# mit-acl/rl_collision_avoidance

Measured on AMD Instinct MI355X. Metric: agent-steps/sec (env.step) at 4 agents x 8192 worlds per GPU, higher is better.
Workload: dtype f64

## Files before the change

### include/cavoid.h

```cpp
#ifndef CAVOID_H
#define CAVOID_H
#include <stdint.h>

#ifdef __cplusplus
extern "C" {
#endif

#define CAVOID_ABI_VERSION 3
#define CAVOID_MAX_ACTIONS 32
#define CAVOID_MAX_AGENTS 64

#define CAVOID_F_AT_GOAL 0x01u
#define CAVOID_F_RAN_OUT 0x02u
#define CAVOID_F_IN_COLL 0x04u
#define CAVOID_F_WAS_AT_GOAL 0x08u
#define CAVOID_F_WAS_IN_COLL 0x10u
#define CAVOID_F_PRESENT 0x20u
#define CAVOID_F_LEARNING 0x40u
#define CAVOID_F_POLICY_SHIFT 8
#define CAVOID_F_POLICY_MASK 7u
enum { CAVOID_POLICY_EXTERNAL = 0, CAVOID_POLICY_STATIC = 1, CAVOID_POLICY_NONCOOP = 2, CAVOID_POLICY_RVO = 3, CAVOID_POLICY_FROZEN_NET = 4 };
#define CAVOID_F_DONE_MASK 0x07u

enum { CAVOID_SORT_CLOSEST_LAST = 0, CAVOID_SORT_CLOSEST_FIRST = 1, CAVOID_SORT_TIME_TO_IMPACT = 2 };
// ... 91 lines not shown
int cavoid_step_autoreset_n(cavoid_env *env, const int32_t *actions, int64_t action_stride, int32_t n_steps, int64_t out_step_stride,
                            float *obs, float *rewards, uint8_t *done, uint8_t *game_over, void *stream);

enum {
    CAVOID_FORM_NONE = 0,
    CAVOID_FORM_STEP = 1,
    CAVOID_FORM_QUAD = 2,
    CAVOID_FORM_RVO = 3,
    CAVOID_FORM_LOOP_PF = 4,
    CAVOID_FORM_LOOP = 5,
    CAVOID_FORM_PIPE = 6,
    CAVOID_FORM_RELAY = 7,
    CAVOID_FORM_CROWD = 8
};
int32_t cavoid_last_step_form(const cavoid_env *env, int32_t *relay_consumers);

int cavoid_step_continuous_autoreset(cavoid_env *env, const float *actions , float *obs, float *rewards, uint8_t *done,
                                     uint8_t *game_over, void *stream);
int cavoid_step_continuous_autoreset_n(cavoid_env *env, const float *actions, int64_t action_stride, int32_t n_steps, int64_t out_step_stride,
                                       float *obs, float *rewards, uint8_t *done, uint8_t *game_over, void *stream);

int32_t cavoid_packed_width(const cavoid_env *env);
int cavoid_reset_packed(cavoid_env *env, const uint8_t *world_mask, float *packed, void *stream);
int cavoid_observe_packed(cavoid_env *env, float *packed, void *stream);
int cavoid_step_packed(cavoid_env *env, const int32_t *actions, float *packed, uint8_t *game_over, void *stream);
int cavoid_step_autoreset_packed(cavoid_env *env, const int32_t *actions, int64_t action_stride, int32_t n_steps, int64_t out_step_stride,
                                 float *packed, uint8_t *game_over, void *stream);
int cavoid_step_continuous_autoreset_packed(cavoid_env *env, const float *actions, int64_t action_stride, int32_t n_steps,
                                            int64_t out_step_stride, float *packed, uint8_t *game_over, void *stream);

// ... 124 lines not shown
```

### rl_collision_avoidance_amd/_lib.py

```python
from __future__ import annotations

import ctypes as C
import os

from .build import LIB_PATH as _DEFAULT_LIB_PATH

LIB_PATH = os.environ.get("CAVOID_LIB", _DEFAULT_LIB_PATH)

MAX_ACTIONS = 32
MAX_AGENTS = 64
TILE_MAX_AGENTS = 16
ABI_VERSION = 3

F_AT_GOAL, F_RAN_OUT, F_IN_COLL, F_WAS_AT_GOAL, F_WAS_IN_COLL, F_PRESENT, F_LEARNING = 1, 2, 4, 8, 16, 32, 64
F_POLICY_SHIFT = 8
F_POLICY_MASK = 7
POLICY_EXTERNAL, POLICY_STATIC, POLICY_NONCOOP, POLICY_RVO, POLICY_FROZEN_NET = 0, 1, 2, 3, 4
F_DONE_MASK = 7
COMM_FORCE_RCCL = 1
STEP_FORMS = ("NONE", "STEP", "QUAD", "RVO", "LOOP_PF", "LOOP", "PIPE", "RELAY", "CROWD")


class CavoidCfg(C.Structure):
    _fields_ = [
# ... 53 lines not shown
        self.code = code


_P = C.c_void_p
SYMBOLS = [
    ("cavoid_abi_version", C.c_int, []),
    ("cavoid_strerror", C.c_char_p, [C.c_int]),
    ("cavoid_last_hip_error", C.c_int, []),
    ("cavoid_default_cfg", C.c_int, [C.POINTER(CavoidCfg), C.c_int32, C.c_int32]),
    ("cavoid_default_actions", C.c_int, [_P, C.POINTER(C.c_int32)]),
    ("cavoid_create", C.c_int, [C.POINTER(CavoidCfg), C.c_int64, C.c_int64, C.c_int, C.POINTER(_P)]),
    ("cavoid_destroy", None, [_P]),
    ("cavoid_num_worlds", C.c_int64, [_P]),
    ("cavoid_obs_width", C.c_int32, [_P]),
    ("cavoid_last_step_form", C.c_int32, [_P, C.POINTER(C.c_int32)]),
    ("cavoid_seed", C.c_int, [_P, C.c_uint64, _P, _P]),
    ("cavoid_get_episode", C.c_int, [_P, _P, _P]),
    ("cavoid_pool_refresh", C.c_int, [_P, C.c_uint32, _P]),
    ("cavoid_set_state", C.c_int, [_P, _P, _P, _P, _P]),
    ("cavoid_get_state", C.c_int, [_P, _P, _P, _P, _P]),
    ("cavoid_reset", C.c_int, [_P, _P, _P, _P]),
    ("cavoid_observe", C.c_int, [_P, _P, _P]),
    ("cavoid_step", C.c_int, [_P, _P, _P, _P, _P, _P, _P]),
    ("cavoid_step_continuous", C.c_int, [_P, _P, _P, _P, _P, _P, _P]),
    ("cavoid_step_autoreset", C.c_int, [_P, _P, _P, _P, _P, _P, _P]),
    ("cavoid_step_autoreset_n", C.c_int, [_P, _P, C.c_int64, C.c_int32, C.c_int64, _P, _P, _P, _P, _P]),
    ("cavoid_step_continuous_autoreset", C.c_int, [_P, _P, _P, _P, _P, _P, _P]),
    ("cavoid_step_continuous_autoreset_n", C.c_int, [_P, _P, C.c_int64, C.c_int32, C.c_int64, _P, _P, _P, _P, _P]),
    ("cavoid_step_continuous_autoreset_packed", C.c_int, [_P, _P, C.c_int64, C.c_int32, C.c_int64, _P, _P, _P]),
    ("cavoid_step_autoreset_n_timed", C.c_int, [_P, _P, C.c_int64, C.c_int32, C.c_int32, C.c_int64, _P, _P, _P, _P, _P, C.POINTER(C.c_float)]),
# ... 73 lines not shown
```

### rl_collision_avoidance_amd/batched_env.py

```python
from __future__ import annotations

import ctypes as C
from typing import Optional, Tuple

import numpy as np
import torch

from . import _lib
from .config import EnvConfig

_SORT = {"closest_last": 0, "closest_first": 1, "time_to_impact": 2}
_DYN = {"unicycle": 0, "unicycle_max_turn_rate": 1, "holonomic": 2}


def make_cfg(config: Optional[EnvConfig] = None, **overrides) -> _lib.CavoidCfg:
    config = config or EnvConfig()
    cfg = _lib.CavoidCfg()
    N = int(config.MAX_NUM_AGENTS_IN_ENVIRONMENT)
    M = int(config.MAX_NUM_OTHER_AGENTS_OBSERVED)
    _lib.check(_lib.lib().cavoid_default_cfg(C.byref(cfg), N, M), "cavoid_default_cfg")
    cfg.dt = config.DT
    cfg.near_goal_threshold = config.NEAR_GOAL_THRESHOLD
    cfg.max_time_ratio = config.MAX_TIME_RATIO
    cfg.collision_dist = config.COLLISION_DIST
# ... 181 lines not shown
    def refresh_pool(self, epoch: int) -> None:
        _lib.check(self._lib.cavoid_pool_refresh(self._h, int(epoch) & 0xFFFFFFFF, self._stream()), "cavoid_pool_refresh")

    @property
    def episode(self) -> torch.Tensor:
        out = torch.empty((self.num_worlds,), dtype=torch.int32, device=self.device)
        _lib.check(self._lib.cavoid_get_episode(self._h, self._ptr(out), self._stream()), "cavoid_get_episode")
        return out

    @property
    def last_step_form(self) -> Tuple[str, int]:
        nc = C.c_int32(0)
        form = self._lib.cavoid_last_step_form(self._h, C.byref(nc))
        return _lib.STEP_FORMS[form], int(nc.value)

    def set_state(self, state_f64: torch.Tensor, state_f32: torch.Tensor, flags: torch.Tensor) -> None:
        A = self.num_worlds * self.max_agents
        f64 = self._want(state_f64, (4, A), torch.float64, "state_f64")
        f32 = self._want(state_f32, (5, A), torch.float32, "state_f32")
        fl = self._want(flags, (A,), torch.int32, "flags")
        _lib.check(self._lib.cavoid_set_state(self._h, self._ptr(f64), self._ptr(f32), self._ptr(fl), self._stream()),
                   "cavoid_set_state")

    def get_state(self) -> Tuple[torch.Tensor, torch.Tensor, torch.Tensor]:
        A = self.num_worlds * self.max_agents
        f64 = torch.empty((4, A), dtype=torch.float64, device=self.device)
        f32 = torch.empty((5, A), dtype=torch.float32, device=self.device)
        fl = torch.empty((A,), dtype=torch.int32, device=self.device)
        _lib.check(self._lib.cavoid_get_state(self._h, self._ptr(f64), self._ptr(f32), self._ptr(fl), self._stream()),
                   "cavoid_get_state")
# ... 164 lines not shown
```

### rl_collision_avoidance_amd/csrc/cavoid_capi.hip

```cpp
#include <hip/hip_runtime.h>
#include <hip/hip_ext.h>

#include <cmath>
#include <cstdlib>
#include <cstring>
#include <new>

#include "cavoid.h"
#include "cavoid_host.hpp"
#include "cavoid_kernels.hpp"
#include "cavoid_launch.hpp"
#include "cavoid_crowd.hpp"

using namespace cavoid;

thread_local int g_last_hip_error = 0;

extern "C" int cavoid_abi_version(void) { return CAVOID_ABI_VERSION; }

extern "C" int cavoid_last_hip_error(void) { return g_last_hip_error; }

extern "C" const char *cavoid_strerror(int code) {
    switch (code) {
        case CAVOID_OK: return "ok";
// ... 312 lines not shown
        return cavoid_launch_rvo(e, MODE, io, s, ev_start, ev_stop);
    if (MODE == MODE_STEP_AUTORESET) {
        const int rc = cavoid_launch_quad(e, io, s, ev_start, ev_stop);
        if (rc != CAVOID_EUNSUPPORTED) return rc;
    }
    const int rc = launch_on<MODE>(e, e->k, e->st, e->grid, io, s, ev_start, ev_stop);
    return stepping ? note_form(e, rc, CAVOID_FORM_STEP) : rc;
}

extern "C" int32_t cavoid_last_step_form(const cavoid_env *e, int32_t *relay_consumers) {
    const int32_t form = e ? e->last_form : CAVOID_FORM_NONE;
    if (relay_consumers) *relay_consumers = form == CAVOID_FORM_RELAY ? e->last_relay_consumers : 0;
    return form;
}

int cavoid_ahead_prepare(cavoid_env *e, int32_t n_steps, hipStream_t s, hipEvent_t *timed_start) {
    if (!e || e->ahead_R <= 0) return CAVOID_OK;
    if (n_steps + 1 > e->ahead_R) return CAVOID_EUNSUPPORTED;
    hipStreamCaptureStatus cap = hipStreamCaptureStatusNone;
    (void)hipStreamIsCapturing(s, &cap);
    const bool capturing = cap != hipStreamCaptureStatusNone;
    if (capturing) e->ahead_always = true;
    if (!e->ahead_always && e->ahead_primed && e->ahead_budget >= n_steps + 1) return CAVOID_OK;
    const int64_t waves = (e->W + e->k.wpw - 1) / e->k.wpw;
    const bool in_place = e->ahead_always;
    const dim3 grid((unsigned)((waves + 3) / 4), in_place ? 1u : (e->ahead_primed ? 4u : 32u)), block(256);
    const uint32_t *hi_in = e->ahead_hi[e->ahead_cur];
    uint32_t *hi_out = e->ahead_hi[in_place ? e->ahead_cur : (e->ahead_cur ^ 1)];
    hipEvent_t ev_fill = (timed_start && !capturing) ? *timed_start : nullptr;
    if (ev_fill) *timed_start = nullptr;
    const int rc = dispatch_n(e->cfg.max_agents, EnvNs{}, [&](auto n) -> int {
        launch_kernel(ahead_fill_kernel<decltype(n)::value>, grid, block, 0, s, ev_fill, nullptr, e->k, e->st.episode, hi_in, hi_out, e->pool, e->ahead_R);
        return CAVOID_OK;
    });
    if (rc != CAVOID_OK) return rc;
    HIP_TRY(hipGetLastError());
    if (!in_place) e->ahead_cur ^= 1;
    if (!capturing) { e->ahead_primed = true; e->ahead_budget = e->ahead_R; }
    return CAVOID_OK;
}
void cavoid_ahead_consumed(cavoid_env *e, int32_t n_steps) {
    if (!e || e->ahead_R <= 0) return;
    e->ahead_budget = e->ahead_budget > n_steps ? e->ahead_budget - n_steps : 0;
}

static int fill_pool(cavoid_env *e, hipStream_t s) {
    if (e->ahead_R > 0) {
        e->ahead_budget = 0;
        e->ahead_primed = false;
        HIP_TRY(hipMemsetAsync(e->ahead_hi[0], 0xFF, 2 * (size_t)e->W * sizeof(uint32_t), s));
        return CAVOID_OK;
    }
    if (e->pool_size <= 0) return CAVOID_OK;
    HIP_TRY(hipMemsetAsync(e->pool_episode, 0xFF, (size_t)e->pool_size * sizeof(uint32_t), s));
    KCfg k = e->k;
    k.num_worlds = e->pool_size;
    k.world_offset = 0;
    k.pool_size = 0;
    KState st{};
// ... 118 lines not shown
    return launch<MODE_STEP>(e, io, static_cast<hipStream_t>(stream));
}

static int launch_autoreset(cavoid_env *e, KIO io, const int32_t *actions, int64_t action_stride, int32_t n_steps, int64_t out_step_stride,
                            hipStream_t s, hipEvent_t ev_start = nullptr, hipEvent_t ev_stop = nullptr, const float *cont = nullptr) {
    if (e->cfg.dynamics == CAVOID_DYN_HOLONOMIC && !cont) return CAVOID_EINVAL;
    if (n_steps < 1 || action_stride < 0) return CAVOID_EINVAL;
    if (cont && n_steps > 1 && action_stride != 0 && action_stride < 2 * e->A) return CAVOID_EINVAL;
    if (out_step_stride != 0 && out_step_stride < e->W) return CAVOID_EINVAL;
    io.out_step_stride = n_steps > 1 ? out_step_stride : 0;
    io.actions = actions;
    io.cont = cont;
    io.action_stride = action_stride;
    io.n_steps = n_steps;
    e->last_form = CAVOID_FORM_NONE;
    if (int rc = cavoid_ahead_prepare(e, n_steps, s, &ev_start)) return rc;
    const int rc = (n_steps > 1 || e->prefetch_single)
                       ? cavoid_launch_multistep(e, io, e->latency_mode != 0, s, ev_start, ev_stop)
                       : launch<MODE_STEP_AUTORESET>(e, io, s, ev_start, ev_stop);
    cavoid_ahead_consumed(e, n_steps);
    return rc;
}

extern "C" int cavoid_step_autoreset(cavoid_env *e, const int32_t *actions, float *obs, float *rew, uint8_t *done, uint8_t *game_over, void *stream) {
    if (step_args(e, actions, rew, done, game_over) != CAVOID_OK) return CAVOID_EINVAL;
    return launch_autoreset(e, plain_io(e, obs, rew, done, game_over), actions, 0, 1, 0, static_cast<hipStream_t>(stream));
}

extern "C" int cavoid_step_autoreset_n(cavoid_env *e, const int32_t *actions, int64_t action_stride, int32_t n_steps, int64_t out_step_stride,
                                       float *obs, float *rew, uint8_t *done, uint8_t *game_over, void *stream) {
    if (step_args(e, actions, rew, done, game_over) != CAVOID_OK || n_steps < 0) return CAVOID_EINVAL;
    if (n_steps == 0) return CAVOID_OK;
    return launch_autoreset(e, plain_io(e, obs, rew, done, game_over), actions, action_stride, n_steps, out_step_stride,
                            static_cast<hipStream_t>(stream));
// ... 119 lines not shown
```

### rl_collision_avoidance_amd/csrc/cavoid_launch.hpp

```cpp
#pragma once
#include <hip/hip_runtime.h>
#include <hip/hip_ext.h>

#include <type_traits>

#include "cavoid.h"
#include "cavoid_host.hpp"
#include "cavoid_kernels.hpp"

struct cavoid_env {
    int device = 0;
    int64_t W = 0, A = 0, world_offset = 0;
    cavoid_cfg cfg{};
    cavoid::KCfg k{};
    cavoid::KState st{};
    cavoid::PoolRec *pool = nullptr;
    uint32_t *pool_episode = nullptr;
    int64_t pool_size = 0;
    int ahead_R = 0;
    uint32_t *ahead_hi[2] = {nullptr, nullptr};
    int ahead_cur = 0;
    int ahead_budget = 0;
    bool ahead_primed = false;
    bool ahead_always = false;
    void *slab = nullptr;
    void *pool_slab = nullptr;
    double *d_actions = nullptr;
    int waves_per_block = 4;
    int grid = 0;
    int pipeline = 2;
    int relay_consumers = 3;
    int latency_mode = 0;
    int quad = -1;
    int prefetch_single = 0;
    int last_form = CAVOID_FORM_NONE;
    int last_relay_consumers = 0;
    hipEvent_t ev0 = nullptr, ev1 = nullptr;
};
// ... 81 lines not shown
    const dim3 grid((unsigned)tiles), block(128);
    const int rc = dispatch_n(e->cfg.max_agents, EnvNs{}, [&](auto n) -> int {
        constexpr int N = decltype(n)::value;
        const size_t lds = pipe_lds_fixed_bytes<N>() + tail;
        if (lds > 65536) return CAVOID_EUNSUPPORTED;
        launch_kernel(env_pipe_kernel<N, RVO>, grid, block, lds, s, ev_start, ev_stop, k, e->st, e->pool, io);
        return CAVOID_OK;
    });
    if (rc != CAVOID_OK) return rc;
    HIP_TRY(hipGetLastError());
    return CAVOID_OK;
}

}

int cavoid_ahead_prepare(cavoid_env *e, int32_t n_steps, hipStream_t s, hipEvent_t *timed_start = nullptr);
void cavoid_ahead_consumed(cavoid_env *e, int32_t n_steps);
int cavoid_launch_relay(cavoid_env *e, const cavoid::KIO &io, hipStream_t s, hipEvent_t ev_start, hipEvent_t ev_stop);
int cavoid_launch_quad(cavoid_env *e, const cavoid::KIO &io, hipStream_t s, hipEvent_t ev_start, hipEvent_t ev_stop);
int cavoid_launch_multistep(cavoid_env *e, const cavoid::KIO &io, bool prefetch, hipStream_t s, hipEvent_t ev_start, hipEvent_t ev_stop);
int cavoid_launch_rvo(cavoid_env *e, int mode, const cavoid::KIO &io, hipStream_t s, hipEvent_t ev_start, hipEvent_t ev_stop);
int cavoid_launch_crowd(cavoid_env *e, int mode, const cavoid::KCfg &k, const cavoid::KState &st, int64_t worlds, const cavoid::KIO &io,
                        hipStream_t s, hipEvent_t ev_start, hipEvent_t ev_stop);
#ifdef CAVOID_TRACE
int cavoid_debug_trace_multistep(unsigned long long *dev_ptr);
int cavoid_debug_trace_rvo(unsigned long long *dev_ptr);
int cavoid_debug_trace_relay(unsigned long long *dev_ptr);
int cavoid_debug_trace_quad(unsigned long long *dev_ptr);
#endif
```

### rl_collision_avoidance_amd/csrc/cavoid_multistep.hip

```cpp
#include "cavoid_launch.hpp"

using namespace cavoid;

int cavoid_launch_multistep(cavoid_env *e, const KIO &io, bool prefetch, hipStream_t s, hipEvent_t ev_start, hipEvent_t ev_stop) {
    if (crowd_form(e->cfg.max_agents))
        return note_form(e, cavoid_launch_crowd(e, MODE_STEP_AUTORESET_N, e->k, e->st, e->W, io, s, ev_start, ev_stop), CAVOID_FORM_CROWD);
    if (e->k.rvo_enabled || (e->k.gen_mode == 1 && e->k.pool_size <= 0))
        return cavoid_launch_rvo(e, prefetch ? MODE_STEP_AUTORESET_PF : MODE_STEP_AUTORESET_N, io, s, ev_start, ev_stop);
    if (prefetch && e->pipeline >= 2 && !io.cont) {
        const int rc = cavoid_launch_relay(e, io, s, ev_start, ev_stop);
        if (rc != CAVOID_EUNSUPPORTED) return rc;
    }
    if (prefetch && e->pipeline && !io.cont) {
        const int rc = launch_pipe<false>(e, io, s, ev_start, ev_stop);
        if (rc != CAVOID_EUNSUPPORTED) return note_form(e, rc, CAVOID_FORM_PIPE);
    }
    if (prefetch) return note_form(e, launch_on<MODE_STEP_AUTORESET_PF>(e, e->k, e->st, e->grid, io, s, ev_start, ev_stop), CAVOID_FORM_LOOP_PF);
    return note_form(e, launch_on<MODE_STEP_AUTORESET_N>(e, e->k, e->st, e->grid, io, s, ev_start, ev_stop), CAVOID_FORM_LOOP);
}

#ifdef CAVOID_TRACE
int cavoid_debug_trace_multistep(unsigned long long *dev_ptr) { return set_trace(dev_ptr); }
#endif
```

### rl_collision_avoidance_amd/csrc/cavoid_relay.hip

```cpp
#include "cavoid_launch.hpp"
#include "cavoid_relay.hpp"

using namespace cavoid;

template <int N>
static int relay_allow_lds() {
    static bool allowed = false;
    if (!allowed) {
        HIP_TRY(hipFuncSetAttribute(reinterpret_cast<const void *>(env_relay_kernel<N>), hipFuncAttributeMaxDynamicSharedMemorySize, (int)kRelayLdsLimit));
        allowed = true;
    }
    return CAVOID_OK;
}

int cavoid_launch_relay(cavoid_env *e, const KIO &io, hipStream_t s, hipEvent_t ev_start, hipEvent_t ev_stop) {
    const KCfg &k = e->k;
    if (k.rvo_enabled || k.pool_size <= 0 || !io.obs || !io.actions || io.cont) return CAVOID_EUNSUPPORTED;
    if (k.switches & kSwSkipDonePairs) return CAVOID_EUNSUPPORTED;
    const int64_t tiles = (e->W + k.wpw - 1) / k.wpw;
    if (tiles > 512) return CAVOID_EUNSUPPORTED;
    if (e->cfg.max_agents > kRelayMaxAgents) return CAVOID_EUNSUPPORTED;
    const int row = io.obs_stride;
    const int tile_floats = (k.tile_rows * row + 3) & ~3;
    if (k.tile_rows < k.wpw * e->cfg.max_agents) return CAVOID_EUNSUPPORTED;
    const dim3 grid((unsigned)tiles);
    int used_nc = 0;
    const int rc = dispatch_n(e->cfg.max_agents, RelayNs{}, [&](auto n) -> int {
        constexpr int N = decltype(n)::value;
        int nc = e->relay_consumers;
        while (nc > 1 && relay_lds_fixed_bytes<N>() + (size_t)nc * tile_floats * sizeof(float) > kRelayLdsLimit) --nc;
        const size_t lds = relay_lds_fixed_bytes<N>() + (size_t)nc * tile_floats * sizeof(float);
        if (lds > kRelayLdsLimit || (nc < 2 && e->relay_consumers >= 2)) return CAVOID_EUNSUPPORTED;
        if (lds > 65536) {
            const int rc_opt = relay_allow_lds<N>();
            if (rc_opt != CAVOID_OK) return rc_opt;
        }
        used_nc = nc;
        launch_kernel(env_relay_kernel<N>, grid, dim3(64 * (3 + nc)), lds, s, ev_start, ev_stop, k, e->st, e->pool, io);
        return CAVOID_OK;
    });
    if (rc != CAVOID_OK) return rc;
    HIP_TRY(hipGetLastError());
    return note_form(e, CAVOID_OK, CAVOID_FORM_RELAY, used_nc);
}

#ifdef CAVOID_TRACE
int cavoid_debug_trace_relay(unsigned long long *dev_ptr) { return set_trace(dev_ptr); }
#endif
```

### rl_collision_avoidance_amd/csrc/cavoid_relay.hpp

```cpp
#pragma once
#include "cavoid_kernels.hpp"

namespace cavoid {

constexpr int kRelayMaxAgents = 6;
template <int N>
__host__ __device__ constexpr int relay_ring() { return N <= 5 ? 8 : 4; }
constexpr size_t kRelayLdsLimit = 80 * 1024;
constexpr int kRelayActRing = 64;
constexpr int kRelayActAhead = 48;
constexpr int kRelayEvq = 8;

struct RelaySeq {
    int spec;
    int stage;
    int res;
    int fin;
    int act;
    int ev;
    int nxt;
    int cons[kRelayMaxConsumers];
    int cfin[kRelayMaxConsumers];
    int coop[2];
    int kernarg[2];
// ... 3 lines not shown
struct RelayTent { double px[64], py[64], vx[64], vy[64], heading[64]; float r[64], gx[64], gy[64], pref[64]; uint32_t flags[64]; };
struct RelayRes { uint32_t flags[64], ctl[64]; float rew[64]; };
struct RelayNxt { double px[64], py[64], heading[64], t_rem[64]; float gx[64], gy[64], radius[64], pref[64]; uint32_t flags[64]; };
#ifndef CAVOID_RELAY_ORDER
#define CAVOID_RELAY_ORDER 0x432150
#endif
#ifndef CAVOID_RELAY_PRIO_D
#define CAVOID_RELAY_PRIO_D 3
#endif
#ifndef CAVOID_RELAY_PRIO_P
#define CAVOID_RELAY_PRIO_P 3
#endif
#ifndef CAVOID_RELAY_PRIO_L
#define CAVOID_RELAY_PRIO_L 0
#endif
#ifndef CAVOID_RELAY_PRIO_C
#define CAVOID_RELAY_PRIO_C 1
#endif
#ifndef CAVOID_RELAY_ABL
#define CAVOID_RELAY_ABL 0
#endif
__device__ __forceinline__ int relay_role_of(int wv, int NC) {
    if (NC == 3) return (int)(((unsigned)CAVOID_RELAY_ORDER >> (4 * wv)) & 15u);
    return wv;
}
constexpr int kRelayCoopWaves = 3;
constexpr int kRelayCoopFromN = 4;
template <int N>
struct RelayCoop {
    static constexpr int K = Others<N>::K;
    uint64_t key[K][64];
    uint32_t bits[K][64];
};
template <int N>
__host__ __device__ constexpr size_t relay_coop_bytes() { return N >= kRelayCoopFromN ? sizeof(RelayCoop<N>) : 0; }
template <int N>
__host__ __device__ constexpr size_t relay_lds_fixed_bytes() {
    return (size_t)lds_floats_block() * sizeof(float) + sizeof(RelaySeq) + kRelayActRing * 64 + relay_ring<N>() * (sizeof(RelayTent) + sizeof(RelayRes)) +
           sizeof(RelayNxt) + kRelayEvq * sizeof(unsigned long long) + relay_coop_bytes<N>();
}

#ifdef CAVOID_TRACE
#define RELAY_STAMP(k)                                                                                         \
    do {                                                                                                       \
        if (lane0 == 0 && g_trace && t == (n_steps >> 1)) g_trace[wave * 32 + (k)] = (unsigned long long)clock64(); \
    } while (0)
#define RELAY_MARK(k)                                                                                          \
    do {                                                                                                       \
        if (lane0 == 0 && g_trace) g_trace[wave * 32 + (k)] = (unsigned long long)clock64();                   \
    } while (0)
#else
#define RELAY_STAMP(k) do { } while (0)
#define RELAY_MARK(k) do { } while (0)
#endif
// ... 184 lines not shown
        gapf[o] = (float)gap_o;
        neighbour_features(e, (float)e.prll_x, (float)e.prll_y, rx, ry, q, feat[o]);
    }
}

struct RelayArgs { KCfg c; KState s; const PoolRec *pool; KIO io; };
template <class T>
__device__ __forceinline__ void relay_load_args(T &dst, const __attribute__((address_space(4))) T *src) {
    static_assert(sizeof(T) % 4 == 0, "whole words");
    const __attribute__((address_space(4))) uint32_t *w = (const __attribute__((address_space(4))) uint32_t *)src;
    uint32_t d[sizeof(T) / 4];
#pragma unroll
    for (int k = 0; k < (int)(sizeof(T) / 4); ++k) d[k] = w[k];
    __builtin_memcpy(&dst, d, sizeof(T));
}
template <int N>
__device__ __forceinline__ void relay_coop_last(unsigned char *smem) {
    unsigned char *sp = smem + lds_floats_block() * sizeof(float);
    RelaySeq *seq = reinterpret_cast<RelaySeq *>(sp); sp += sizeof(RelaySeq) + kRelayEvq * sizeof(unsigned long long);
    const unsigned long long kp = (unsigned long long)(uint32_t)relay_peek(&seq->kernarg[0]) | ((unsigned long long)(uint32_t)relay_peek(&seq->kernarg[1]) << 32);
    typedef const __attribute__((address_space(4))) RelayArgs *ArgP;
    const ArgP ka = (ArgP)kp;
    KCfg c;
    KIO io;
    relay_load_args(c, &ka->c);
    relay_load_args(io, &ka->io);
    RelayTent *tents = reinterpret_cast<RelayTent *>(sp); sp += relay_ring<N>() * sizeof(RelayTent) + sizeof(RelayNxt);
    RelayRes *ress = reinterpret_cast<RelayRes *>(sp); sp += relay_ring<N>() * sizeof(RelayRes) + kRelayActRing * 64;
    RelayCoop<N> *coopb = reinterpret_cast<RelayCoop<N> *>(sp); sp += relay_coop_bytes<N>();
    float *tiles = reinterpret_cast<float *>(sp);
    const int lane0 = threadIdx.x & 63;
    const int NC = (blockDim.x >> 6) - 3;
    const int role = relay_role_of(threadIdx.x >> 6, NC);
    const int pw = role < 2 ? role : 2;
    const int ostride = io.obs_stride;
    const int tile_floats = (c.tile_rows * ostride + 3) & ~3;
    const int wpw = c.wpw, lanes_used = wpw * N;
    const int64_t wave = relay_peek(&seq->tile_id);
    const int64_t w0 = wave * wpw;
    const int lw = lane0 / N, i0 = lane0 - lw * N;
    const int64_t w = w0 + lw;
    const bool active = lane0 < lanes_used && w < c.num_worlds;
// ... 61 lines not shown
        const bool lines = ((rows_active * ostride) & 31) == 0 && (reinterpret_cast<uintptr_t>(dst) & 127) == 0;
        if (io.out_step_stride != 0 && lines) flush_tile<4, true, true>(tile, dst, rows_active * ostride, pw * 64 + lane0, 64 * kRelayCoopWaves);
        else if (io.out_step_stride != 0) flush_tile<4, true>(tile, dst, rows_active * ostride, pw * 64 + lane0, 64 * kRelayCoopWaves);
        else flush_tile<4>(tile, dst, rows_active * ostride, pw * 64 + lane0, 64 * kRelayCoopWaves);
    }
    if (pw == 0 && active) {
        if (!packed) {
            io.rew[slot_w * N + a_idx0] = rew_c;
            io.done[slot_w * N + a_idx0] = (ctl_c & 1u) ? 1 : 0;
        }
        if (i0 == 0) io.game_over[slot_w + w] = (ctl_c & 2u) ? 1 : 0;
    }
    if (pw == 0) RELAY_MARK(29);
}

template <int N>
__global__ void __launch_bounds__(64 * (3 + kRelayMaxConsumers), 1) env_relay_kernel(const KCfg c, const KState s, const PoolRec *pool, const KIO io) {
    extern __shared__ __attribute__((aligned(16))) unsigned char smem[];
    unsigned char *sp = smem;
    double *lds_tab = reinterpret_cast<double *>(sp); sp += lds_floats_block() * sizeof(float);
    RelaySeq *seq = reinterpret_cast<RelaySeq *>(sp); sp += sizeof(RelaySeq);
    unsigned long long *evq = reinterpret_cast<unsigned long long *>(sp); sp += kRelayEvq * sizeof(unsigned long long);
    RelayTent *tents = reinterpret_cast<RelayTent *>(sp); sp += relay_ring<N>() * sizeof(RelayTent);
    RelayNxt *nbuf = reinterpret_cast<RelayNxt *>(sp); sp += sizeof(RelayNxt);
    RelayRes *ress = reinterpret_cast<RelayRes *>(sp); sp += relay_ring<N>() * sizeof(RelayRes);
    unsigned char *actring = sp; sp += kRelayActRing * 64;
    RelayCoop<N> *coopb = reinterpret_cast<RelayCoop<N> *>(sp); sp += relay_coop_bytes<N>();
    float *tiles = reinterpret_cast<float *>(sp);

    const int NC = (blockDim.x >> 6) - 3;
    const int role = relay_role_of(threadIdx.x >> 6, NC);
    const int lane0 = threadIdx.x & 63;
    const int ostride = io.obs_stride;
    const int tile_floats = (c.tile_rows * ostride + 3) & ~3;
    const int wpw = c.wpw, lanes_used = wpw * N;
    const int64_t wave = blockIdx.x;
    const int64_t w0 = wave * wpw;
    const int lw = lane0 / N, i0 = lane0 - lw * N;
    const int64_t w = w0 + lw;
    const bool active = lane0 < lanes_used && w < c.num_worlds;
    const int base0 = lane0 < lanes_used ? lw * N : 0;
    const int64_t a_idx0 = w * N + i0;
    const bool packed = io.packed != 0;
    int64_t worlds_here = c.num_worlds - w0;
    if (worlds_here > wpw) worlds_here = wpw;
    if (worlds_here < 0) worlds_here = 0;
    const int n_steps = io.n_steps;
    constexpr bool kCoop = N >= kRelayCoopFromN;
    const bool coop_role = role < 2 || role == 2 + NC;

    if (role == 0 && lane0 < (int)(sizeof(RelaySeq) / sizeof(int))) reinterpret_cast<int *>(seq)[lane0] = 0;
    if constexpr (kCoop) {
        if (role == 0 && lane0 == 0) {
            const unsigned long long kp = (unsigned long long)__builtin_amdgcn_kernarg_segment_ptr();
            seq->kernarg[0] = (int)(uint32_t)kp; seq->kernarg[1] = (int)(uint32_t)(kp >> 32);
            seq->tile_id = (int)blockIdx.x;
        }
    }

    if (role == 0) {
        __builtin_amdgcn_s_setprio(CAVOID_RELAY_PRIO_D);
        RELAY_MARK(20);
        KCfg cd = c;
        asm volatile("" : "+s"(cd.dt), "+s"(cd.near_goal_sq), "+s"(cd.actions_fp32), "+s"(cd.dynamics),
                     "+s"(cd.timeout_enabled), "+s"(cd.switches));
        const RelayTrig trig = relay_trig_constants();
        Agent a;
// ... 70 lines not shown
            if (CAVOID_RARE((posted >> 1) < t + 1 - ((CAVOID_RELAY_ABL & 16) ? 1 : 0)))
                do posted = relay_peek(&seq->res); while ((posted >> 1) < t + 1 - ((CAVOID_RELAY_ABL & 16) ? 1 : 0));
            asm volatile("" ::: "memory");
            RELAY_STAMP(2);
            moved_any = moved_any || T_moving;
            const bool surprise = !(CAVOID_RELAY_ABL & 24) && (posted >> 1) == t + 1 && (posted & 1) != 0;
            if (CAVOID_RARE(surprise)) {
                const uint32_t vflags = *(relay_lds_u32 *)&res->flags[lane], ctl = *(relay_lds_u32 *)&res->ctl[lane];
                const bool restart = (ctl & 2u) != 0u;
                const unsigned long long rmask = __ballot(restart);
                Agent S = T;
                S.flags = vflags;
                if (rmask != 0ull) {
                    relay_wait(&seq->nxt, events + 1);
                    Agent nx;
                    relay_read_nxt(*nbuf, lane, nx);
                    bool mr;
                    const RelayStatics ksn = relay_statics(nx, active);
                    const Agent Tr = relay_advance(cd, trig, nx, ksn, tab_s1, tab_h1, active, mr);
                    if (restart) {
                        S = nx; episode += 1u; restarted_any = true; Tn = Tr; mn = mr; ks = ksn;
                        stage_out(tents[t & (relay_ring<N>() - 1)], nx, ksn.r_staged, lane);
                        res->flags[lane] = nx.flags;
                    }
                }
                const bool s_present = active && (S.flags & CAVOID_F_PRESENT);
                const bool s_done = (S.flags & CAVOID_F_DONE_MASK) != 0u;
                const bool frozen = s_present && s_done && !restart;
                uint32_t fflags = S.flags;
                if (S.flags & CAVOID_F_AT_GOAL) fflags |= CAVOID_F_WAS_AT_GOAL;
                if (S.flags & CAVOID_F_IN_COLL) fflags |= CAVOID_F_WAS_IN_COLL;
                Tn.px = frozen ? S.px : Tn.px; Tn.py = frozen ? S.py : Tn.py; Tn.heading = frozen ? S.heading : Tn.heading;
                Tn.t_rem = frozen ? S.t_rem : Tn.t_rem;
                Tn.vx = frozen ? 0.0 : Tn.vx; Tn.vy = frozen ? 0.0 : Tn.vy; Tn.speed = frozen ? 0.0f : Tn.speed;
                Tn.flags = frozen ? fflags : Tn.flags;
                mn = frozen ? false : mn;
                stage_out(tn, Tn, ks.r_staged, lane);
                relay_post(&seq->stage, t + 2);
                if (rmask != 0ull) {
                    relay_wait(&seq->nxt, events + 1 - (kRelayEvq - 1));
                    if (lane == 0) evq[events & (kRelayEvq - 1)] = rmask;
                    events += 1;
                    relay_post(&seq->ev, events);
                }
            }
            T = Tn;
            T_moving = mn;
            tab_s = tab_s2; tab_h = tab_h2;
            act_q = act3;
            relay_post(&seq->fin, t + 1);
            RELAY_STAMP(3);
        }
        Agent S = T;
        {
            const int t = n_steps - 1;
            relay_spin(&seq->res, 2 * (t + 1));
            RelayRes *res = &ress[t & (relay_ring<N>() - 1)];
            const uint32_t vflags = res->flags[lane0], ctl = res->ctl[lane0];
            moved_any = moved_any || T_moving;
            S.flags = vflags;
            const bool restart = (ctl & 2u) != 0u;
            if (__ballot(restart) != 0ull) {
                relay_wait(&seq->nxt, events + 1);
                Agent nx;
                relay_read_nxt(*nbuf, lane0, nx);
                if (restart) {
                    S = nx; episode += 1u; restarted_any = true;
                    stage_out(tents[t & (relay_ring<N>() - 1)], nx, relay_statics(nx, active).r_staged, lane0);
                    res->flags[lane0] = nx.flags;
                }
            }
            relay_post(&seq->fin, t + 1);
        }
        RELAY_MARK(23);
        relay_post(&seq->stage, n_steps + 1);
        if (restarted_any) {
            store_agent(s, a_idx0, S);
            if (i0 == 0) s.episode[w] = episode;
        } else if (present_first) {
            if (moved_any) {
// ... 83 lines not shown
                    const int sidx = loaded + q < upto ? loaded + q : upto - 1;
                    v[q] = io.actions[(int64_t)sidx * io.action_stride + a_safe];
                }
#pragma unroll
                for (int q = 0; q < 8; ++q) {
                    int x = v[q] < 0 ? 0 : (v[q] >= c.num_actions ? c.num_actions - 1 : v[q]);
                    if (loaded + q < upto) actring[((loaded + q) & (kRelayActRing - 1)) * 64 + lane0] = (unsigned char)x;
                }
                loaded = loaded + 8 < upto ? loaded + 8 : upto;
            }
        };
        load_actions(n_steps < 8 ? n_steps : 8);
        RELAY_MARK(26);
        __syncthreads();
        relay_post(&seq->act, loaded);
        {
            Agent r0;
            absent_agent(r0);
            if (active) load_pool(pool, (int64_t)pool_index(c, (uint32_t)(c.world_offset + w), ep + 1u) * N + i0, r0);
            RelayNxt &nb = *nbuf;
            nb.px[lane0] = r0.px; nb.py[lane0] = r0.py; nb.heading[lane0] = r0.heading; nb.t_rem[lane0] = r0.t_rem;
            nb.gx[lane0] = r0.gx; nb.gy[lane0] = r0.gy; nb.radius[lane0] = r0.radius; nb.pref[lane0] = r0.pref;
            nb.flags[lane0] = r0.flags;
            relay_post(&seq->nxt, 1);
            RELAY_MARK(27);
        }
        int served = 0, idle_polls = 0;
        while (true) {
            const int ev = relay_peek(&seq->ev), fin = relay_peek(&seq->fin);
            if (served < ev) {
                asm volatile("" ::: "memory");
                const unsigned long long mask = evq[served & (kRelayEvq - 1)];
                if ((mask >> lane0) & 1ull) {
                    ep += 1u;
                    Agent r0;
                    load_pool(pool, (int64_t)pool_index(c, (uint32_t)(c.world_offset + w), ep + 1u) * N + i0, r0);
                    RelayNxt &nb = *nbuf;
                    nb.px[lane0] = r0.px; nb.py[lane0] = r0.py; nb.heading[lane0] = r0.heading; nb.t_rem[lane0] = r0.t_rem;
                    nb.gx[lane0] = r0.gx; nb.gy[lane0] = r0.gy; nb.radius[lane0] = r0.radius; nb.pref[lane0] = r0.pref;
                    nb.flags[lane0] = r0.flags;
                }
                served += 1;
                idle_polls = 0;
                relay_post(&seq->nxt, served + 1);
                continue;
            }
            if (loaded < n_steps && loaded < fin + kRelayActAhead) {
                int upto = fin + kRelayActAhead;
                if (upto > loaded + 8) upto = loaded + 8;
                if (upto > n_steps) upto = n_steps;
                load_actions(upto);
                idle_polls = 0;
                relay_post(&seq->act, loaded);
                continue;
            }
            if (fin >= n_steps && relay_peek(&seq->stage) > n_steps) break;
            if (++idle_polls > kRelayPollLimit) __builtin_trap();
            __builtin_amdgcn_s_sleep(2);
        }
// ... 47 lines not shown
                    io.rew[slot_w * N + a_idx0] = rew_c;
                    io.done[slot_w * N + a_idx0] = (ctl_c & 1u) ? 1 : 0;
                }
                if (i0 == 0) io.game_over[slot_w + w] = (ctl_c & 2u) ? 1 : 0;
            }
            relay_post(&seq->cons[cid], t + 1);
            RELAY_STAMP(19);
            if (t == 0) RELAY_MARK(28);
            if (t == n_steps - 1) RELAY_MARK(29);
        }
        __builtin_amdgcn_s_waitcnt(0);
        if (cid == 0) RELAY_MARK(30);
        relay_post(&seq->cfin[cid], 1);
    }
    if constexpr (kCoop) {
        if (coop_role) relay_coop_last<N>(smem);
    }
}

}
```

Before: 23.62 billion.

## Generate next-episode agents inside relay loader wave instead of reading ahead ring

```diff
diff --git a/include/cavoid.h b/include/cavoid.h
--- a/include/cavoid.h
+++ b/include/cavoid.h
@@ -129,6 +129,7 @@
     CAVOID_FORM_CROWD = 8
 };
 int32_t cavoid_last_step_form(const cavoid_env *env, int32_t *relay_consumers);
+int64_t cavoid_ahead_refills(const cavoid_env *env);
 
 int cavoid_step_continuous_autoreset(cavoid_env *env, const float *actions , float *obs, float *rewards, uint8_t *done,
                                      uint8_t *game_over, void *stream);
diff --git a/rl_collision_avoidance_amd/_lib.py b/rl_collision_avoidance_amd/_lib.py
--- a/rl_collision_avoidance_amd/_lib.py
+++ b/rl_collision_avoidance_amd/_lib.py
@@ -91,6 +91,7 @@
     ("cavoid_num_worlds", C.c_int64, [_P]),
     ("cavoid_obs_width", C.c_int32, [_P]),
     ("cavoid_last_step_form", C.c_int32, [_P, C.POINTER(C.c_int32)]),
+    ("cavoid_ahead_refills", C.c_int64, [_P]),
     ("cavoid_seed", C.c_int, [_P, C.c_uint64, _P, _P]),
     ("cavoid_get_episode", C.c_int, [_P, _P, _P]),
     ("cavoid_pool_refresh", C.c_int, [_P, C.c_uint32, _P]),
diff --git a/rl_collision_avoidance_amd/batched_env.py b/rl_collision_avoidance_amd/batched_env.py
--- a/rl_collision_avoidance_amd/batched_env.py
+++ b/rl_collision_avoidance_amd/batched_env.py
@@ -219,6 +219,10 @@
         form = self._lib.cavoid_last_step_form(self._h, C.byref(nc))
         return _lib.STEP_FORMS[form], int(nc.value)
 
+    @property
+    def ahead_refills(self) -> int:
+        return int(self._lib.cavoid_ahead_refills(self._h))
+
     def set_state(self, state_f64: torch.Tensor, state_f32: torch.Tensor, flags: torch.Tensor) -> None:
         A = self.num_worlds * self.max_agents
         f64 = self._want(state_f64, (4, A), torch.float64, "state_f64")
diff --git a/rl_collision_avoidance_amd/csrc/cavoid_capi.hip b/rl_collision_avoidance_amd/csrc/cavoid_capi.hip
--- a/rl_collision_avoidance_amd/csrc/cavoid_capi.hip
+++ b/rl_collision_avoidance_amd/csrc/cavoid_capi.hip
@@ -350,13 +350,14 @@
     return form;
 }
 
-int cavoid_ahead_prepare(cavoid_env *e, int32_t n_steps, hipStream_t s, hipEvent_t *timed_start) {
+int cavoid_ahead_prepare(cavoid_env *e, int32_t n_steps, hipStream_t s, hipEvent_t *timed_start, bool reads_ring) {
     if (!e || e->ahead_R <= 0) return CAVOID_OK;
     if (n_steps + 1 > e->ahead_R) return CAVOID_EUNSUPPORTED;
     hipStreamCaptureStatus cap = hipStreamCaptureStatusNone;
     (void)hipStreamIsCapturing(s, &cap);
     const bool capturing = cap != hipStreamCaptureStatusNone;
     if (capturing) e->ahead_always = true;
+    if (!reads_ring) return CAVOID_OK;
     if (!e->ahead_always && e->ahead_primed && e->ahead_budget >= n_steps + 1) return CAVOID_OK;
     const int64_t waves = (e->W + e->k.wpw - 1) / e->k.wpw;
     const bool in_place = e->ahead_always;
@@ -371,6 +372,7 @@
     });
     if (rc != CAVOID_OK) return rc;
     HIP_TRY(hipGetLastError());
+    e->ahead_refills += 1;
     if (!in_place) e->ahead_cur ^= 1;
     if (!capturing) { e->ahead_primed = true; e->ahead_budget = e->ahead_R; }
     return CAVOID_OK;
@@ -379,6 +381,8 @@
     if (!e || e->ahead_R <= 0) return;
     e->ahead_budget = e->ahead_budget > n_steps ? e->ahead_budget - n_steps : 0;
 }
+
+extern "C" int64_t cavoid_ahead_refills(const cavoid_env *e) { return e ? e->ahead_refills : 0; }
 
 static int fill_pool(cavoid_env *e, hipStream_t s) {
     if (e->ahead_R > 0) {
@@ -527,10 +531,18 @@
     io.action_stride = action_stride;
     io.n_steps = n_steps;
     e->last_form = CAVOID_FORM_NONE;
-    if (int rc = cavoid_ahead_prepare(e, n_steps, s, &ev_start)) return rc;
-    const int rc = (n_steps > 1 || e->prefetch_single)
-                       ? cavoid_launch_multistep(e, io, e->latency_mode != 0, s, ev_start, ev_stop)
-                       : launch<MODE_STEP_AUTORESET>(e, io, s, ev_start, ev_stop);
+    const bool loop = n_steps > 1 || e->prefetch_single;
+    const bool generates = loop && cavoid_multistep_takes_relay(e, io, e->latency_mode != 0) && cavoid_relay_generates(e);
+    if (int rc = cavoid_ahead_prepare(e, n_steps, s, &ev_start, !generates)) return rc;
+    int rc = CAVOID_EUNSUPPORTED;
+    if (generates) {
+        rc = cavoid_launch_relay(e, io, s, ev_start, ev_stop);
+        if (rc == CAVOID_EUNSUPPORTED)
+            if (int rc_a = cavoid_ahead_prepare(e, n_steps, s, &ev_start)) return rc_a;
+    }
+    if (rc == CAVOID_EUNSUPPORTED)
+        rc = loop ? cavoid_launch_multistep(e, io, e->latency_mode != 0, s, ev_start, ev_stop, !generates)
+                  : launch<MODE_STEP_AUTORESET>(e, io, s, ev_start, ev_stop);
     cavoid_ahead_consumed(e, n_steps);
     return rc;
 }
diff --git a/rl_collision_avoidance_amd/csrc/cavoid_launch.hpp b/rl_collision_avoidance_amd/csrc/cavoid_launch.hpp
--- a/rl_collision_avoidance_amd/csrc/cavoid_launch.hpp
+++ b/rl_collision_avoidance_amd/csrc/cavoid_launch.hpp
@@ -22,6 +22,7 @@
     int ahead_cur = 0;
     int ahead_budget = 0;
     bool ahead_primed = false;
+    int64_t ahead_refills = 0;
     bool ahead_always = false;
     void *slab = nullptr;
     void *pool_slab = nullptr;
@@ -133,11 +134,15 @@
 
 }
 
-int cavoid_ahead_prepare(cavoid_env *e, int32_t n_steps, hipStream_t s, hipEvent_t *timed_start = nullptr);
+int cavoid_ahead_prepare(cavoid_env *e, int32_t n_steps, hipStream_t s, hipEvent_t *timed_start = nullptr, bool reads_ring = true);
 void cavoid_ahead_consumed(cavoid_env *e, int32_t n_steps);
 int cavoid_launch_relay(cavoid_env *e, const cavoid::KIO &io, hipStream_t s, hipEvent_t ev_start, hipEvent_t ev_stop);
+bool cavoid_relay_eligible(const cavoid_env *e, const cavoid::KIO &io, int *nc_out);
+bool cavoid_relay_generates(const cavoid_env *e);
 int cavoid_launch_quad(cavoid_env *e, const cavoid::KIO &io, hipStream_t s, hipEvent_t ev_start, hipEvent_t ev_stop);
-int cavoid_launch_multistep(cavoid_env *e, const cavoid::KIO &io, bool prefetch, hipStream_t s, hipEvent_t ev_start, hipEvent_t ev_stop);
+int cavoid_launch_multistep(cavoid_env *e, const cavoid::KIO &io, bool prefetch, hipStream_t s, hipEvent_t ev_start, hipEvent_t ev_stop,
+                            bool try_relay = true);
+bool cavoid_multistep_takes_relay(const cavoid_env *e, const cavoid::KIO &io, bool prefetch);
 int cavoid_launch_rvo(cavoid_env *e, int mode, const cavoid::KIO &io, hipStream_t s, hipEvent_t ev_start, hipEvent_t ev_stop);
 int cavoid_launch_crowd(cavoid_env *e, int mode, const cavoid::KCfg &k, const cavoid::KState &st, int64_t worlds, const cavoid::KIO &io,
                         hipStream_t s, hipEvent_t ev_start, hipEvent_t ev_stop);
diff --git a/rl_collision_avoidance_amd/csrc/cavoid_multistep.hip b/rl_collision_avoidance_amd/csrc/cavoid_multistep.hip
--- a/rl_collision_avoidance_amd/csrc/cavoid_multistep.hip
+++ b/rl_collision_avoidance_amd/csrc/cavoid_multistep.hip
@@ -2,12 +2,17 @@
 
 using namespace cavoid;
 
-int cavoid_launch_multistep(cavoid_env *e, const KIO &io, bool prefetch, hipStream_t s, hipEvent_t ev_start, hipEvent_t ev_stop) {
+bool cavoid_multistep_takes_relay(const cavoid_env *e, const KIO &io, bool prefetch) {
+    if (crowd_form(e->cfg.max_agents) || e->k.rvo_enabled || (e->k.gen_mode == 1 && e->k.pool_size <= 0)) return false;
+    return prefetch && e->pipeline >= 2 && !io.cont && cavoid_relay_eligible(e, io, nullptr);
+}
+
+int cavoid_launch_multistep(cavoid_env *e, const KIO &io, bool prefetch, hipStream_t s, hipEvent_t ev_start, hipEvent_t ev_stop, bool try_relay) {
     if (crowd_form(e->cfg.max_agents))
         return note_form(e, cavoid_launch_crowd(e, MODE_STEP_AUTORESET_N, e->k, e->st, e->W, io, s, ev_start, ev_stop), CAVOID_FORM_CROWD);
     if (e->k.rvo_enabled || (e->k.gen_mode == 1 && e->k.pool_size <= 0))
         return cavoid_launch_rvo(e, prefetch ? MODE_STEP_AUTORESET_PF : MODE_STEP_AUTORESET_N, io, s, ev_start, ev_stop);
-    if (prefetch && e->pipeline >= 2 && !io.cont) {
+    if (try_relay && prefetch && e->pipeline >= 2 && !io.cont) {
         const int rc = cavoid_launch_relay(e, io, s, ev_start, ev_stop);
         if (rc != CAVOID_EUNSUPPORTED) return rc;
     }
diff --git a/rl_collision_avoidance_amd/csrc/cavoid_relay.hip b/rl_collision_avoidance_amd/csrc/cavoid_relay.hip
--- a/rl_collision_avoidance_amd/csrc/cavoid_relay.hip
+++ b/rl_collision_avoidance_amd/csrc/cavoid_relay.hip
@@ -1,42 +1,71 @@
+#include <atomic>
+
 #include "cavoid_launch.hpp"
 #include "cavoid_relay.hpp"
 
 using namespace cavoid;
 
-template <int N>
+template <int N, bool GEN>
 static int relay_allow_lds() {
-    static bool allowed = false;
-    if (!allowed) {
-        HIP_TRY(hipFuncSetAttribute(reinterpret_cast<const void *>(env_relay_kernel<N>), hipFuncAttributeMaxDynamicSharedMemorySize, (int)kRelayLdsLimit));
-        allowed = true;
+    constexpr int kDevices = 64;
+    static std::atomic<bool> allowed[kDevices];
+    int dev = -1;
+    if (hipGetDevice(&dev) != hipSuccess) { (void)hipGetLastError(); return CAVOID_EUNSUPPORTED; }
+    if (dev >= 0 && dev < kDevices && allowed[dev].load(std::memory_order_acquire)) return CAVOID_OK;
+    if (hipFuncSetAttribute(reinterpret_cast<const void *>(env_relay_kernel<N, GEN>), hipFuncAttributeMaxDynamicSharedMemorySize,
+                            (int)kRelayLdsLimit) != hipSuccess) {
+        (void)hipGetLastError();
+        return CAVOID_EUNSUPPORTED;
     }
+    if (dev >= 0 && dev < kDevices) allowed[dev].store(true, std::memory_order_release);
     return CAVOID_OK;
 }
 
+bool cavoid_relay_eligible(const cavoid_env *e, const KIO &io, int *nc_out) {
+    const KCfg &k = e->k;
+    if (k.rvo_enabled || k.pool_size <= 0 || !io.obs || !io.actions || io.cont) return false;
+    if (k.switches & kSwSkipDonePairs) return false;
+    const int64_t tiles = (e->W + k.wpw - 1) / k.wpw;
+    if (tiles > 512) return false;
+    if (e->cfg.max_agents > kRelayMaxAgents) return false;
+    const int tile_floats = (k.tile_rows * io.obs_stride + 3) & ~3;
+    if (k.tile_rows < k.wpw * e->cfg.max_agents) return false;
+    int used_nc = 0;
+    const bool gen = cavoid_relay_generates(e);
+    const int rc = dispatch_n(e->cfg.max_agents, RelayNs{}, [&](auto n) -> int {
+        constexpr int N = decltype(n)::value;
+        const size_t fixed = gen ? relay_lds_fixed_bytes<N, true>() : relay_lds_fixed_bytes<N, false>();
+        int nc = e->relay_consumers;
+        while (nc > 1 && fixed + (size_t)nc * tile_floats * sizeof(float) > kRelayLdsLimit) --nc;
+        const size_t lds = fixed + (size_t)nc * tile_floats * sizeof(float);
+        if (lds > kRelayLdsLimit || (nc < 2 && e->relay_consumers >= 2)) return CAVOID_EUNSUPPORTED;
+        used_nc = nc;
+        return CAVOID_OK;
+    });
+    if (rc != CAVOID_OK) return false;
+    if (nc_out) *nc_out = used_nc;
+    return true;
+}
+
+bool cavoid_relay_generates(const cavoid_env *e) { return e->ahead_R > 0 && e->k.gen_mode == 0; }
+
 int cavoid_launch_relay(cavoid_env *e, const KIO &io, hipStream_t s, hipEvent_t ev_start, hipEvent_t ev_stop) {
     const KCfg &k = e->k;
-    if (k.rvo_enabled || k.pool_size <= 0 || !io.obs || !io.actions || io.cont) return CAVOID_EUNSUPPORTED;
-    if (k.switches & kSwSkipDonePairs) return CAVOID_EUNSUPPORTED;
+    int used_nc = 0;
+    if (!cavoid_relay_eligible(e, io, &used_nc)) return CAVOID_EUNSUPPORTED;
     const int64_t tiles = (e->W + k.wpw - 1) / k.wpw;
-    if (tiles > 512) return CAVOID_EUNSUPPORTED;
-    if (e->cfg.max_agents > kRelayMaxAgents) return CAVOID_EUNSUPPORTED;
-    const int row = io.obs_stride;
-    const int tile_floats = (k.tile_rows * row + 3) & ~3;
-    if (k.tile_rows < k.wpw * e->cfg.max_agents) return CAVOID_EUNSUPPORTED;
-    const dim3 grid((unsigned)tiles);
-    int used_nc = 0;
+    const int tile_floats = (k.tile_rows * io.obs_stride + 3) & ~3;
+    const dim3 grid((unsigned)tiles), block(64 * (3 + used_nc));
+    const bool gen = cavoid_relay_generates(e);
     const int rc = dispatch_n(e->cfg.max_agents, RelayNs{}, [&](auto n) -> int {
         constexpr int N = decltype(n)::value;
-        int nc = e->relay_consumers;
-        while (nc > 1 && relay_lds_fixed_bytes<N>() + (size_t)nc * tile_floats * sizeof(float) > kRelayLdsLimit) --nc;
-        const size_t lds = relay_lds_fixed_bytes<N>() + (size_t)nc * tile_floats * sizeof(float);
-        if (lds > kRelayLdsLimit || (nc < 2 && e->relay_consumers >= 2)) return CAVOID_EUNSUPPORTED;
+        const size_t lds = (gen ? relay_lds_fixed_bytes<N, true>() : relay_lds_fixed_bytes<N, false>()) + (size_t)used_nc * tile_floats * sizeof(float);
         if (lds > 65536) {
-            const int rc_opt = relay_allow_lds<N>();
+            const int rc_opt = gen ? relay_allow_lds<N, true>() : relay_allow_lds<N, false>();
             if (rc_opt != CAVOID_OK) return rc_opt;
         }
-        used_nc = nc;
-        launch_kernel(env_relay_kernel<N>, grid, dim3(64 * (3 + nc)), lds, s, ev_start, ev_stop, k, e->st, e->pool, io);
+        if (gen) launch_kernel(env_relay_kernel<N, true>, grid, block, lds, s, ev_start, ev_stop, k, e->st, e->pool, io);
+        else launch_kernel(env_relay_kernel<N, false>, grid, block, lds, s, ev_start, ev_stop, k, e->st, e->pool, io);
         return CAVOID_OK;
     });
     if (rc != CAVOID_OK) return rc;
diff --git a/rl_collision_avoidance_amd/csrc/cavoid_relay.hpp b/rl_collision_avoidance_amd/csrc/cavoid_relay.hpp
--- a/rl_collision_avoidance_amd/csrc/cavoid_relay.hpp
+++ b/rl_collision_avoidance_amd/csrc/cavoid_relay.hpp
@@ -41,6 +41,9 @@
 #ifndef CAVOID_RELAY_PRIO_L
 #define CAVOID_RELAY_PRIO_L 0
 #endif
+#ifndef CAVOID_RELAY_PRIO_LGEN
+#define CAVOID_RELAY_PRIO_LGEN 0
+#endif
 #ifndef CAVOID_RELAY_PRIO_C
 #define CAVOID_RELAY_PRIO_C 1
 #endif
@@ -61,10 +64,16 @@
 };
 template <int N>
 __host__ __device__ constexpr size_t relay_coop_bytes() { return N >= kRelayCoopFromN ? sizeof(RelayCoop<N>) : 0; }
-template <int N>
+#ifndef CAVOID_RELAY_GEN_DEPTH
+#define CAVOID_RELAY_GEN_DEPTH 2
+#endif
+template <bool GEN>
+__host__ __device__ constexpr int relay_nxt_depth() { return GEN ? CAVOID_RELAY_GEN_DEPTH : 1; }
+static_assert(CAVOID_RELAY_GEN_DEPTH == 1 || CAVOID_RELAY_GEN_DEPTH == 2, "a power of two, below the event queue's depth");
+template <int N, bool GEN = false>
 __host__ __device__ constexpr size_t relay_lds_fixed_bytes() {
     return (size_t)lds_floats_block() * sizeof(float) + sizeof(RelaySeq) + kRelayActRing * 64 + relay_ring<N>() * (sizeof(RelayTent) + sizeof(RelayRes)) +
-           sizeof(RelayNxt) + kRelayEvq * sizeof(unsigned long long) + relay_coop_bytes<N>();
+           relay_nxt_depth<GEN>() * sizeof(RelayNxt) + kRelayEvq * sizeof(unsigned long long) + relay_coop_bytes<N>();
 }
 
 #ifdef CAVOID_TRACE
@@ -279,7 +288,7 @@
     for (int k = 0; k < (int)(sizeof(T) / 4); ++k) d[k] = w[k];
     __builtin_memcpy(&dst, d, sizeof(T));
 }
-template <int N>
+template <int N, bool GEN>
 __device__ __forceinline__ void relay_coop_last(unsigned char *smem) {
     unsigned char *sp = smem + lds_floats_block() * sizeof(float);
     RelaySeq *seq = reinterpret_cast<RelaySeq *>(sp); sp += sizeof(RelaySeq) + kRelayEvq * sizeof(unsigned long long);
@@ -290,7 +299,7 @@
     KIO io;
     relay_load_args(c, &ka->c);
     relay_load_args(io, &ka->io);
-    RelayTent *tents = reinterpret_cast<RelayTent *>(sp); sp += relay_ring<N>() * sizeof(RelayTent) + sizeof(RelayNxt);
+    RelayTent *tents = reinterpret_cast<RelayTent *>(sp); sp += relay_ring<N>() * sizeof(RelayTent) + relay_nxt_depth<GEN>() * sizeof(RelayNxt);
     RelayRes *ress = reinterpret_cast<RelayRes *>(sp); sp += relay_ring<N>() * sizeof(RelayRes) + kRelayActRing * 64;
     RelayCoop<N> *coopb = reinterpret_cast<RelayCoop<N> *>(sp); sp += relay_coop_bytes<N>();
     float *tiles = reinterpret_cast<float *>(sp);
@@ -382,7 +391,7 @@
     if (pw == 0) RELAY_MARK(29);
 }
 
-template <int N>
+template <int N, bool GEN = false>
 __global__ void __launch_bounds__(64 * (3 + kRelayMaxConsumers), 1) env_relay_kernel(const KCfg c, const KState s, const PoolRec *pool, const KIO io) {
     extern __shared__ __attribute__((aligned(16))) unsigned char smem[];
     unsigned char *sp = smem;
@@ -390,7 +399,8 @@
     RelaySeq *seq = reinterpret_cast<RelaySeq *>(sp); sp += sizeof(RelaySeq);
     unsigned long long *evq = reinterpret_cast<unsigned long long *>(sp); sp += kRelayEvq * sizeof(unsigned long long);
     RelayTent *tents = reinterpret_cast<RelayTent *>(sp); sp += relay_ring<N>() * sizeof(RelayTent);
-    RelayNxt *nbuf = reinterpret_cast<RelayNxt *>(sp); sp += sizeof(RelayNxt);
+    RelayNxt *nbuf = reinterpret_cast<RelayNxt *>(sp); sp += relay_nxt_depth<GEN>() * sizeof(RelayNxt);
+    constexpr uint32_t kNxtMask = (uint32_t)relay_nxt_depth<GEN>() - 1u;
     RelayRes *ress = reinterpret_cast<RelayRes *>(sp); sp += relay_ring<N>() * sizeof(RelayRes);
     unsigned char *actring = sp; sp += kRelayActRing * 64;
     RelayCoop<N> *coopb = reinterpret_cast<RelayCoop<N> *>(sp); sp += relay_coop_bytes<N>();
@@ -418,7 +428,7 @@
     const bool coop_role = role < 2 || role == 2 + NC;
 
     if (role == 0 && lane0 < (int)(sizeof(RelaySeq) / sizeof(int))) reinterpret_cast<int *>(seq)[lane0] = 0;
-    if constexpr (kCoop) {
+    if constexpr (kCoop || GEN) {
         if (role == 0 && lane0 == 0) {
             const unsigned long long kp = (unsigned long long)__builtin_amdgcn_kernarg_segment_ptr();
             seq->kernarg[0] = (int)(uint32_t)kp; seq->kernarg[1] = (int)(uint32_t)(kp >> 32);
@@ -519,7 +529,7 @@
                 if (rmask != 0ull) {
                     relay_wait(&seq->nxt, events + 1);
                     Agent nx;
-                    relay_read_nxt(*nbuf, lane, nx);
+                    relay_read_nxt(nbuf[(episode + 1u) & kNxtMask], lane, nx);
                     bool mr;
                     const RelayStatics ksn = relay_statics(nx, active);
                     const Agent Tr = relay_advance(cd, trig, nx, ksn, tab_s1, tab_h1, active, mr);
@@ -543,7 +553,7 @@
                 stage_out(tn, Tn, ks.r_staged, lane);
                 relay_post(&seq->stage, t + 2);
                 if (rmask != 0ull) {
-                    relay_wait(&seq->nxt, events + 1 - (kRelayEvq - 1));
+                    relay_wait(&seq->nxt, events + 1 - (kRelayEvq - 1) + (relay_nxt_depth<GEN>() - 1));
                     if (lane == 0) evq[events & (kRelayEvq - 1)] = rmask;
                     events += 1;
                     relay_post(&seq->ev, events);
@@ -568,7 +578,7 @@
             if (__ballot(restart) != 0ull) {
                 relay_wait(&seq->nxt, events + 1);
                 Agent nx;
-                relay_read_nxt(*nbuf, lane0, nx);
+                relay_read_nxt(nbuf[(episode + 1u) & kNxtMask], lane0, nx);
                 if (restart) {
                     S = nx; episode += 1u; restarted_any = true;
                     stage_out(tents[t & (relay_ring<N>() - 1)], nx, relay_statics(nx, active).r_staged, lane0);
@@ -682,7 +692,26 @@
         RELAY_MARK(26);
         __syncthreads();
         relay_post(&seq->act, loaded);
-        {
+        KCfg cg;
+        if constexpr (GEN) {
+            const unsigned long long kp = (unsigned long long)(uint32_t)relay_peek(&seq->kernarg[0]) | ((unsigned long long)(uint32_t)relay_peek(&seq->kernarg[1]) << 32);
+            relay_load_args(cg, &((const __attribute__((address_space(4))) RelayArgs *)kp)->c);
+        }
+        if constexpr (GEN) {
+            for (uint32_t d = 1; d <= (uint32_t)relay_nxt_depth<GEN>(); ++d) {
+                Agent r0;
+                absent_agent(r0);
+                __builtin_amdgcn_s_setprio(CAVOID_RELAY_PRIO_LGEN);
+                if (active) generate_agent<N>(cg, (uint32_t)(cg.world_offset + w), ep + d, i0, r0);
+                __builtin_amdgcn_s_setprio(CAVOID_RELAY_PRIO_L);
+                RelayNxt &nb = nbuf[(ep + d) & kNxtMask];
+                nb.px[lane0] = r0.px; nb.py[lane0] = r0.py; nb.heading[lane0] = r0.heading; nb.t_rem[lane0] = r0.t_rem;
+                nb.gx[lane0] = r0.gx; nb.gy[lane0] = r0.gy; nb.radius[lane0] = r0.radius; nb.pref[lane0] = r0.pref;
+                nb.flags[lane0] = r0.flags;
+                relay_post(&seq->nxt, (int)d);
+                if (d == 1) RELAY_MARK(27);
+            }
+        } else {
             Agent r0;
             absent_agent(r0);
             if (active) load_pool(pool, (int64_t)pool_index(c, (uint32_t)(c.world_offset + w), ep + 1u) * N + i0, r0);
@@ -699,18 +728,21 @@
             if (served < ev) {
                 asm volatile("" ::: "memory");
                 const unsigned long long mask = evq[served & (kRelayEvq - 1)];
+                if constexpr (GEN) __builtin_amdgcn_s_setprio(CAVOID_RELAY_PRIO_LGEN);
                 if ((mask >> lane0) & 1ull) {
                     ep += 1u;
                     Agent r0;
-                    load_pool(pool, (int64_t)pool_index(c, (uint32_t)(c.world_offset + w), ep + 1u) * N + i0, r0);
-                    RelayNxt &nb = *nbuf;
+                    if constexpr (GEN) generate_agent<N>(cg, (uint32_t)(cg.world_offset + w), ep + (uint32_t)relay_nxt_depth<GEN>(), i0, r0);
+                    else load_pool(pool, (int64_t)pool_index(c, (uint32_t)(c.world_offset + w), ep + 1u) * N + i0, r0);
+                    RelayNxt &nb = nbuf[ep & kNxtMask];
                     nb.px[lane0] = r0.px; nb.py[lane0] = r0.py; nb.heading[lane0] = r0.heading; nb.t_rem[lane0] = r0.t_rem;
                     nb.gx[lane0] = r0.gx; nb.gy[lane0] = r0.gy; nb.radius[lane0] = r0.radius; nb.pref[lane0] = r0.pref;
                     nb.flags[lane0] = r0.flags;
                 }
                 served += 1;
                 idle_polls = 0;
-                relay_post(&seq->nxt, served + 1);
+                relay_post(&seq->nxt, served + relay_nxt_depth<GEN>());
+                if constexpr (GEN) __builtin_amdgcn_s_setprio(CAVOID_RELAY_PRIO_L);
                 continue;
             }
             if (loaded < n_steps && loaded < fin + kRelayActAhead) {
@@ -788,8 +820,8 @@
         relay_post(&seq->cfin[cid], 1);
     }
     if constexpr (kCoop) {
-        if (coop_role) relay_coop_last<N>(smem);
-    }
-}
-
-}
+        if (coop_role) relay_coop_last<N, GEN>(smem);
+    }
+}
+
+}
```

New measurement: 23.11 billion. 0.979x the previous value.
